# ERGO-Code/ipx

Hardware: AMD Instinct MI355X
Metric: kkt_solves_per_sec (higher is better)
Workload: dtype f64; 1 GPU; C3 synthetic LP m=1000000 n=2000000 8 nnz/col (nnz=16000000), KKTSolverDiag::Solve = diag-precond CR to tol=0.3*sqrt(mu), scaling spread s=1; rows of AI partitioned over 1 GPU(s); errflag=0

## Files before the change

ipx_amd/csrc/internal.hpp:

```cpp
#pragma once

#include <hip/hip_runtime.h>

#include <chrono>
#include <cstdint>
#include <cstdio>
#include <cstdlib>
#include <algorithm>
#include <cstring>
#include <functional>
#include <memory>
#include <stdexcept>
#include <string>
#include <type_traits>
#include <vector>

#include "../../include/ipx_kkt_hip.h"

namespace ipxk {

struct Error : std::runtime_error {
    int code;
    Error(int c, const std::string& what) : std::runtime_error(what), code(c) {}
};
// ... 77 lines not shown
    int64_t g = (n + kBlock - 1) / kBlock;
    if (g < 1) g = 1;
    return (int)(g < cap ? g : cap);
}
inline int vec_grid(int64_t len) { return grid_for(len, 1024); }

struct GatherView {
    int nrows, ncols;
    int P, G, RT, Q;
    int RWrows;
    const int* step_ptr;
    const int* wg_chunk_ptr;
    const int* chunk_start;
    const int* chunk_info;
    const int* chunk_step;
    const unsigned char* counts;
    const int* idx;
    const double* val;
    const unsigned char* row_long;
    int nseg;
    const int* seg_p0;
    const int* seg_p1;
    const int* lidx;
    const double* lval;
    int nlong;
    const int* long_row;
    const int* long_slot;
    double* long_partials;
    unsigned long long* stamps;
    int masked;
};

constexpr int kSlicedRows = 1024;
constexpr int kSlicedMaxTile = 7680;

struct SlicedView {
    int nrows, nrows_pad, nslices, nrb;
    int R;
    const unsigned* tile_ptr;
    const unsigned char* cnt;
    const int* idx;
    const double* val;
    double* partial;
    const unsigned char* row_long;
    int masked;
};

struct SlicedMatrix {
    bool built = false;
    int nslices = 0, nrb = 0, nrows_pad = 0, max_tile = 0, R = kSlicedRows;
    double dominant_fraction = 1.0;
    DevBuf<unsigned> tile_ptr;
    DevBuf<unsigned char> cnt;
    DevBuf<int> idx;
    DevBuf<double> val, partial;
};

constexpr int kSortedThreads = 256;
constexpr int kSortedMaxSub = 8192;
constexpr int kSortedOffBits = 18;
struct SortedView {
    int nrows, nrows_pad, nslices, nsub, nrb, RB, slice_elems;
    const int* xmin;
    const unsigned char* row_long;
    const unsigned* sub_ptr;
    const unsigned char* cnt;
    const unsigned* pack;
    const double* val;
    double* partial;
};
struct SortedMatrix {
    bool built = false;
    int nslices = 0, nsub = 0, nrb = 0, RB = 0, nrows_pad = 0, max_sub = 0, slice_elems = 0;
    DevBuf<unsigned> sub_ptr, pack;
    DevBuf<unsigned char> cnt;
    DevBuf<double> val, partial;
    bool fused = false;
    DevBuf<int> xmin;
};

constexpr int kAccThreads = 512;
constexpr int kAccPerThread = 4;
constexpr int kAccBatch = kAccThreads * kAccPerThread;
constexpr int kAccMaxRows = 16384;
struct AccView {
    int nrows, nrows_pad, nslices, nrb, RB, slice_elems;
    const int* xmin;
    const unsigned* tile_batch;
    const unsigned* bptr;
    const unsigned* pack;
    const double* val;
    double* partial;
};
struct AccMatrix {
    bool built = false;
    int nslices = 0, nrb = 0, RB = 0, nrows_pad = 0, slice_elems = 0;
    int64_t nbatches = 0, deferred = 0;
    DevBuf<unsigned> tile_batch, bptr, pack;
    DevBuf<double> val, partial;
    bool fused = false;
    DevBuf<int> xmin;
};

struct LayoutScratch;

enum class SpmvLayout { phased, sliced, fused, sorted, sortedfused, acc, plain, accfused };
constexpr int kNumSpmvLayouts = 8;
inline constexpr const char* kSpmvLayoutNames[kNumSpmvLayouts] = {"phased", "sliced", "fused", "sorted", "sortedfused", "acc", "plain",
                                                                  "accfused"};

inline int combine_grid_for(int64_t nrows) {
    static const int cap = [] { const char* e = getenv("IPXK_COMBINE_GRID"); return e && atoi(e) > 0 ? std::min(atoi(e), 1024) : 1024; }();
    return (int)std::min<int64_t>(cap, std::max<int64_t>(1, (nrows + kBlock - 1) / kBlock));
}

struct GatherMatrix {
    int nrows = 0, ncols = 0;
    int64_t nnz = 0;
    int P = 1, G = 1, RT = 1, Q = 1, RWrows = kBlock;
    DevBuf<int> step_ptr, idx, wg_chunk_ptr, chunk_start, chunk_info, chunk_step;
    DevBuf<unsigned char> counts, row_long;
    DevBuf<double> val;
    int nseg = 0, nlong = 0;
    DevBuf<int> seg_p0, seg_p1, lidx, long_row, long_slot;
    DevBuf<double> lval, long_partials;
    DevBuf<unsigned long long> stamps;
    int tune_level = 2;
    bool keep_plain = false;
    std::vector<int> h_plain_ptr;
    DevBuf<int> plain_idx;
    DevBuf<double> plain_val;

    void build(int64_t nrows_, int64_t ncols_, const ipxint* hptr, const ipxint* hidx,
               const double* hval, hipStream_t s);
    bool build_device(LayoutScratch& S, int64_t nrows_, int64_t ncols_, int64_t nnz_, const int* dptr, const int* didx,
                      const double* dval, hipStream_t s);
    bool build_device_local(LayoutScratch& S, int64_t nrows_, int64_t ncols_, int64_t nnz_, const int* dptr, const int* didx,
                            const double* dval, double share, hipStream_t s);
    void set_geometry(int64_t nrows_, int64_t ncols_);
    SpmvLayout layout = SpmvLayout::phased;
    SpmvLayout tile_base() const { return !sliced.built ? SpmvLayout::phased : sliced.nslices == 1 ? SpmvLayout::fused : SpmvLayout::sliced; }
    float tuned_us[kNumSpmvLayouts] = {};
    float time_layout(SpmvLayout L, hipStream_t s);
    void select_layout(const std::function<bool(SpmvLayout)>& make, hipStream_t s);
    SlicedMatrix sliced;
    SortedMatrix sorted;
    void build_sorted(const ipxint* hptr, const ipxint* hidx, const double* hval, hipStream_t s);
    void build_sorted_fused(const ipxint* hptr, const ipxint* hidx, const double* hval, hipStream_t s);
    AccMatrix acc;
    void build_acc(const ipxint* hptr, const ipxint* hidx, const double* hval, hipStream_t s);
    void build_acc_fused(const ipxint* hptr, const ipxint* hidx, const double* hval, hipStream_t s);
    AccMatrix accf;
    AccView acc_fused_view() const;
    AccView acc_view() const;
    const int* csr_ptr = nullptr;
    const int* csr_idx = nullptr;
    const double* csr_val = nullptr;
    int plain_grid() const { return (int)std::min<int64_t>(kMaxPartials, std::max<int64_t>(1, ((int64_t)nrows * 8 + kBlock - 1) / kBlock)); }
    int sorted_fused_grid() const {
        static const int cap = [] { const char* e = getenv("IPXK_SF_GRID"); return e && atoi(e) > 0 ? std::min(atoi(e), kMaxPartials) : kMaxPartials; }();
        return std::min(sorted.nrb, cap);
    }
    SortedView sorted_view() const;
    void build_sliced(const ipxint* hptr, const ipxint* hidx, const double* hval, hipStream_t s, int ns_request);
    SlicedView sliced_view(int which = 0) const;
    int fused_grid() const { return std::min(sliced.nrb, kMaxPartials); }
// ... 154 lines not shown
```

ipx_amd/csrc/layout_device.hip:

```cpp
#include <numeric>
#include <rocprim/device/device_radix_sort.hpp>
#include <rocprim/device/device_scan.hpp>

#include "layout_scratch.hpp"

namespace ipxk {

template <class K>
void sort_pairs(Tmp& T, const K* kin, K* kout, const unsigned* vin, unsigned* vout, size_t n, int bits, hipStream_t s) {
    size_t bytes = 0;
    IPXK_HIP(rocprim::radix_sort_pairs(nullptr, bytes, kin, kout, vin, vout, n, 0u, (unsigned)bits, s));
    IPXK_HIP(rocprim::radix_sort_pairs(T.need(bytes), bytes, kin, kout, vin, vout, n, 0u, (unsigned)bits, s));
}
template void sort_pairs<unsigned>(Tmp&, const unsigned*, unsigned*, const unsigned*, unsigned*, size_t, int, hipStream_t);
template void sort_pairs<u64>(Tmp&, const u64*, u64*, const unsigned*, unsigned*, size_t, int, hipStream_t);
void sort_keys(Tmp& T, u64* in, u64* out, size_t n, hipStream_t s) {
    size_t bytes = 0;
    IPXK_HIP(rocprim::radix_sort_keys(nullptr, bytes, in, out, n, 0u, 64u, s));
    IPXK_HIP(rocprim::radix_sort_keys(T.need(bytes), bytes, in, out, n, 0u, 64u, s));
}
void scan_int(Tmp& T, const int* in, int* out, size_t n, hipStream_t s) {
    size_t bytes = 0;
    IPXK_HIP(rocprim::exclusive_scan(nullptr, bytes, in, out, 0, n, rocprim::plus<int>(), s));
    IPXK_HIP(rocprim::exclusive_scan(T.need(bytes), bytes, in, out, 0, n, rocprim::plus<int>(), s));
// ... 99 lines not shown
                                u64* __restrict__ key, unsigned* __restrict__ pos, int* __restrict__ rowof) {
    IPXK_GRID_STRIDE(r, nrows) {
        const u64 tile0 = (u64)(r / RB) * (u64)ns;
        for (int p = ptr[r]; p < ptr[r + 1]; p++) {
            const int sl = idx[p] / slice, off = idx[p] - sl * slice;
            key[p] = ((tile0 + (u64)sl) << kSortedOffBits) | (u64)(unsigned)off;
            pos[p] = (unsigned)p;
            rowof[p] = (int)r;
        }
    }
}
__global__ void acc_words_kernel(int64_t nz, const u64* __restrict__ keys, const unsigned* __restrict__ perm, const int* __restrict__ rowof, int RB,
                                 unsigned* __restrict__ word) {
    IPXK_GRID_STRIDE(e, nz) word[e] = ((unsigned)(rowof[perm[e]] % RB) << kSortedOffBits) | (unsigned)(keys[e] & ((1u << kSortedOffBits) - 1u));
}
__global__ __launch_bounds__(64) void acc_batch_kernel(int RB, const unsigned* __restrict__ tile_ptr, const unsigned* __restrict__ word,
                                                        unsigned* __restrict__ dst, unsigned* pendA, unsigned* pendB, unsigned* __restrict__ bstart,
                                                        unsigned* __restrict__ nbatch, u64* deferred_total) {
    extern __shared__ unsigned ab_lds[];
    unsigned* stamp = ab_lds;
    unsigned* claim = ab_lds + RB;
    const int tile = blockIdx.x, lane = threadIdx.x;
    const unsigned e0 = tile_ptr[tile];
    const int ne = (int)(tile_ptr[tile + 1] - e0);
    for (int r = lane; r < RB; r += 64) { stamp[r] = 0u; claim[r] = 0xffffffffu; }
    __syncthreads();
    unsigned cur = 1;
    int fill = 0, out = 0, nb = 0, cursor = 0, na = 0, ia = 0, nbp = 0;
    u64 ndef = 0;
    unsigned *pa = pendA + e0, *pb = pendB + e0;
    if (ne > 0) { if (lane == 0) bstart[e0] = e0; nb = 1; }
    const u64 lt = (1ull << lane) - 1ull;
    while (out < ne) {
        int n = 0, c = 0;
        if (ia < na) {
            n = min(64, na - ia);
            if (lane < n) c = (int)__hip_atomic_load(pa + ia + lane, __ATOMIC_RELAXED, __HIP_MEMORY_SCOPE_AGENT);
            ia += n;
        } else if (fill < kAccBatch && cursor < ne) {
            n = min(64, ne - cursor);
            c = cursor + lane;
            cursor += n;
        } else {
            if (lane == 0) bstart[e0 + nb] = e0 + (unsigned)out;
            nb++; cur++; fill = 0;
            unsigned* t = pa; pa = pb; pb = t;
            na = nbp; ia = 0; nbp = 0;
            __syncthreads();
            continue;
        }
        const bool live = lane < n;
        const unsigned row = live ? (word[e0 + c] >> kSortedOffBits) : 0u;
        const bool ok = live && stamp[row] != cur;
        if (ok) atomicMin(&claim[row], (unsigned)lane);
        __syncthreads();
        const bool win = ok && claim[row] == (unsigned)lane;
        __syncthreads();
        if (win) { claim[row] = 0xffffffffu; stamp[row] = cur; }
        const u64 wmask = __ballot(win);
        const int prefix = __popcll(wmask & lt);
        const bool take = win && prefix < kAccBatch - fill;
        if (take) dst[e0 + c] = e0 + (unsigned)(out + prefix);
        const int nt = __popcll(__ballot(take));
        const bool def = live && !take;
        const u64 dmask = __ballot(def);
        if (def) pb[nbp + __popcll(dmask & lt)] = (unsigned)c;
        const int nd = __popcll(dmask);
        nbp += nd; ndef += (u64)nd; out += nt; fill += nt;
        __syncthreads();
    }
    if (lane == 0) {
        nbatch[tile] = (unsigned)nb;
        if (ndef) atomicAdd(deferred_total, ndef);
    }
}
__global__ void acc_scatter_kernel(int64_t nz, const unsigned* __restrict__ dst, const unsigned* __restrict__ word, const unsigned* __restrict__ perm,
                                   const double* __restrict__ val, unsigned* __restrict__ pack, double* __restrict__ out_val) {
    IPXK_GRID_STRIDE(e, nz) {
        const unsigned d = dst[e];
        pack[d] = word[e];
        out_val[d] = val[perm[e]];
    }
}
__global__ void acc_bptr_kernel(int ntiles, const unsigned* __restrict__ tile_ptr, const unsigned* __restrict__ tile_batch,
                                const unsigned* __restrict__ bstart, unsigned nz, unsigned* __restrict__ bptr) {
    const int tile = blockIdx.x;
    if (tile >= ntiles) return;
    const unsigned e0 = tile_ptr[tile], b0 = tile_batch[tile], nb = tile_batch[tile + 1] - b0;
    for (unsigned q = threadIdx.x; q < nb; q += blockDim.x) bptr[b0 + q] = bstart[e0 + q];
    if (tile == ntiles - 1 && threadIdx.x == 0) bptr[tile_batch[ntiles]] = nz;
}

__global__ void tile_window_kernel(int nrows, const int* __restrict__ ptr, const int* __restrict__ idx, int RB, int* __restrict__ lo,
                                   int* __restrict__ hi, unsigned char* __restrict__ cnt, int* flags) {
    IPXK_GRID_STRIDE(r, nrows) {
        const int p0 = ptr[r], p1 = ptr[r + 1];
        if (cnt) { if (p1 - p0 > 255) flags[0] = 1; cnt[r] = (unsigned char)(p1 - p0); }
        if (p1 == p0) continue;
        int a = idx[p0], b = a;
        for (int p = p0 + 1; p < p1; p++) {
            const int v = idx[p];
            if (v <= idx[p - 1]) flags[1] = 1;
            a = min(a, v); b = max(b, v);
        }
        atomicMin(lo + r / RB, a);
        atomicMax(hi + r / RB, b);
    }
}
__global__ void tile_window_stats_kernel(int nrb, int nrows, int RB, const int* __restrict__ ptr, int* __restrict__ lo, const int* __restrict__ hi,
                                         int* out) {
    IPXK_GRID_STRIDE(t, nrb) {
        const int r0 = (int)t * RB, r1 = min(nrows, r0 + RB);
        const int ne = ptr[r1] - ptr[r0];
        if (ne == 0) { lo[t] = 0; continue; }
        atomicMax(out + 0, hi[t] - lo[t]);
        atomicMax(out + 1, ne);
    }
}
__global__ void fused_keys_kernel(int nrows, const int* __restrict__ ptr, const int* __restrict__ idx, int RB, const int* __restrict__ lo,
                                  u64* __restrict__ key, unsigned* __restrict__ pos, int* __restrict__ rowof) {
    IPXK_GRID_STRIDE(r, nrows) {
        const u64 t = (u64)(r / RB);
        const int base = lo[r / RB];
        for (int p = ptr[r]; p < ptr[r + 1]; p++) {
            key[p] = (t << kSortedOffBits) | (u64)(unsigned)(idx[p] - base);
            pos[p] = (unsigned)p;
            if (rowof) rowof[p] = (int)r;
        }
    }
}
__global__ void sorted_fused_fill_kernel(int64_t nz, const u64* __restrict__ keys, const unsigned* __restrict__ perm, const int* __restrict__ ptr, int RB,
                                         const double* __restrict__ val, unsigned* __restrict__ pack, double* __restrict__ out_val) {
    IPXK_GRID_STRIDE(f, nz) {
        const u64 k = keys[f];
        const unsigned p = perm[f], t = (unsigned)(k >> kSortedOffBits);
        pack[f] = ((p - (unsigned)ptr[(size_t)t * RB]) << kSortedOffBits) | (unsigned)(k & ((1u << kSortedOffBits) - 1u));
        out_val[f] = val[p];
    }
}
__global__ void tile_ptr_from_rows_kernel(int nrb, int nrows, int RB, const int* __restrict__ ptr, unsigned* __restrict__ out) {
    IPXK_GRID_STRIDE(t, (int64_t)nrb + 1) out[t] = (unsigned)ptr[min((int64_t)nrows, t * RB)];
}
}

namespace {
constexpr int kMaxLongRowsDevice = 1 << 16;
__global__ void long_flag_kernel(int nrows, const int* __restrict__ ptr, unsigned char* __restrict__ flag, int* __restrict__ slen, int* counters,
                                 int* __restrict__ list, int cap) {
    IPXK_GRID_STRIDE(r, (int64_t)nrows + 1) {
        if (r == nrows) { slen[r] = 0; continue; }
        const int len = ptr[r + 1] - ptr[r];
        const bool lg = len > kMaxRowLen;
        flag[r] = lg ? 1 : 0;
        slen[r] = lg ? 0 : len;
        if (lg) {
            const int k = atomicAdd(counters, 1);
            if (k < cap) list[k] = (int)r;
        }
    }
}
__global__ void strip_copy_kernel(int nrows, const int* __restrict__ ptr, const int* __restrict__ sptr, const unsigned char* __restrict__ flag,
                                  const int* __restrict__ idx, const double* __restrict__ val, int* __restrict__ oidx, double* __restrict__ oval) {
    const int g = threadIdx.x & 7;
    for (int64_t r = ((int64_t)blockIdx.x * blockDim.x + threadIdx.x) >> 3; r < nrows; r += ((int64_t)gridDim.x * blockDim.x) >> 3) {
        if (flag[r]) continue;
        const int p0 = ptr[r], len = ptr[r + 1] - p0, q0 = sptr[r];
// ... 134 lines not shown
    for (;; search.next()) {
        RB = search.rows;
        if (search.gave_up()) return false;
        nrb = (nrows + RB - 1) / RB;
        nsubs = (int64_t)nrb * ns * nsub;
        if ((u64)nsubs * (u64)RB >= (u64(1) << 32)) return false;
        hipLaunchKernelGGL(sorted_keys1_kernel, dim3(gridn(nrows)), dim3(kBlock), 0, s, nrows, dptr, didx, RB, ns, nsub, (int)slice, (int)half,
                           S.k1.get(), S.v1.get());
        sort_pairs<unsigned>(S.T, S.k1.get(), S.k2.get(), S.v1.get(), S.v2.get(), nz, bits_for((u64)nsubs * (u64)RB - 1), s);
        out.sub_ptr.ensure((size_t)nsubs + 1);
        hipLaunchKernelGGL(lower_bounds_kernel<unsigned>, dim3(gridn(nsubs + 1)), dim3(kBlock), 0, s, nsubs + 1, nnz, S.k2.get(), (u64)RB, 0,
                           out.sub_ptr.get());
        IPXK_HIP(hipMemsetAsync(S.stats.get(), 0, 8 * sizeof(int), s));
        hipLaunchKernelGGL(max_range_kernel, dim3(gridn(nsubs)), dim3(kBlock), 0, s, nsubs, out.sub_ptr.get(), S.stats.get());
        IPXK_HIP(hipMemcpyAsync(&max_sub, S.stats.get(), sizeof(int), hipMemcpyDeviceToHost, s));
        IPXK_HIP(hipStreamSynchronize(s));
        if (search.fits(max_sub)) break;
    }
    const size_t nslots = (size_t)nsubs * RB;
    out.cnt.ensure(nslots); out.pack.ensure(nz); out.val.ensure(nz);
    IPXK_HIP(hipMemsetAsync(out.cnt.get(), 0, nslots, s));
    IPXK_HIP(hipMemsetAsync(S.stats.get(), 0, 8 * sizeof(int), s));
    hipLaunchKernelGGL(run_counts_kernel, dim3(gridn(nnz)), dim3(kBlock), 0, s, nnz, S.k2.get(), out.cnt.get(), S.stats.get());
    hipLaunchKernelGGL(sorted_keys2_kernel, dim3(gridn(nnz)), dim3(kBlock), 0, s, nnz, S.k2.get(), S.v2.get(), didx, RB, ns, nsub, (int)slice,
                       S.q1.get(), S.v3.get());
    sort_pairs<u64>(S.T, S.q1.get(), S.q2.get(), S.v3.get(), S.v4.get(), nz, kSortedOffBits + bits_for((u64)nsubs - 1), s);
    hipLaunchKernelGGL(sorted_fill_kernel, dim3(gridn(nnz)), dim3(kBlock), 0, s, nnz, S.q2.get(), S.v4.get(), S.v2.get(), out.sub_ptr.get(), dval,
                       out.pack.get(), out.val.get());
    int over = 0;
    IPXK_HIP(hipMemcpyAsync(&over, S.stats.get(), sizeof(int), hipMemcpyDeviceToHost, s));
    IPXK_HIP(hipStreamSynchronize(s));
    IPXK_HIP(hipGetLastError());
    if (over) { out = SortedMatrix(); return false; }
    out.nslices = ns; out.nsub = nsub; out.nrb = nrb; out.RB = RB; out.nrows_pad = nrb * RB;
    out.max_sub = max_sub; out.slice_elems = (int)slice;
    out.partial.resize((size_t)ns * out.nrows_pad);
    out.built = true;
    return true;
}

int acc_persist_grid(int ns) {
    static const int setting = [] { const char* e = getenv("IPXK_ACC_PERSIST"); return e ? std::max(0, atoi(e)) : 1; }();
    if (setting == 0 || ns < 1) return 0;
    static int cus[64] = {};
    int dev = 0;
    IPXK_HIP(hipGetDevice(&dev));
    if (dev < 0 || dev >= 64) dev = 0;
    if (cus[dev] == 0) IPXK_HIP(hipDeviceGetAttribute(&cus[dev], hipDeviceAttributeMultiprocessorCount, dev));
    const int L = std::lcm(8, ns);
    const int n = setting > 1 ? std::min(setting, cus[dev]) : cus[dev];
    return std::max(L, n / L * L);
}

int acc_rows_per_block(int nrows, int ns) {
    static const int cap = [] { const char* e = getenv("IPXK_ACC_ROWS"); return e && atoi(e) >= 1024 ? std::min(atoi(e), kAccMaxRows) & ~1 : kAccMaxRows; }();
    static const bool balance = !(getenv("IPXK_ACC_BALANCE") && getenv("IPXK_ACC_BALANCE")[0] == '0');
    if (const int G = balance ? acc_persist_grid(ns) : 0) {
        const int64_t per = G / ns;
        const int64_t nrb = (((int64_t)nrows + cap - 1) / cap + per - 1) / per * per;
        int rb = (int)(((int64_t)nrows + nrb - 1) / nrb);
        rb += rb & 1;
        if (rb >= 1024 && 8 * (int64_t)rb >= 7 * (int64_t)cap) return rb;
    }
    int RB = cap;
    while (RB > 1024 && ((int64_t)nrows + RB - 1) / RB * (int64_t)ns < 256) RB /= 2;
    return RB;
}

struct AccTemps {
    DevBuf<int> rowof;
    DevBuf<unsigned> tile_ptr, nbatch, bstart;
    AccTemps(int64_t ntiles, size_t nz) : rowof(nz), tile_ptr((size_t)ntiles + 1), nbatch((size_t)ntiles + 1), bstart(nz) {}
};
static void acc_batches(LayoutScratch& S, AccMatrix& out, AccTemps& T, int64_t ntiles, int RB, int64_t nnz, const double* dval, hipStream_t s) {
    const size_t nz = (size_t)nnz;
    unsigned* word = S.k1.get();
    hipLaunchKernelGGL(acc_words_kernel, dim3(gridn(nnz)), dim3(kBlock), 0, s, nnz, S.q2.get(), S.v2.get(), T.rowof.get(), RB, word);
    IPXK_HIP(hipMemsetAsync(S.stats.get(), 0, 8 * sizeof(int), s));
    const size_t lds = (size_t)RB * 2 * sizeof(unsigned);
    IPXK_HIP(hipFuncSetAttribute(reinterpret_cast<const void*>(acc_batch_kernel), hipFuncAttributeMaxDynamicSharedMemorySize,
                                 (int)(kAccMaxRows * 2 * sizeof(unsigned))));
    hipLaunchKernelGGL(acc_batch_kernel, dim3((unsigned)ntiles), dim3(64), lds, s, RB, T.tile_ptr.get(), word, S.k2.get(), S.v3.get(), S.v4.get(),
                       T.bstart.get(), T.nbatch.get(), reinterpret_cast<u64*>(S.stats.get()));
    out.tile_batch.ensure((size_t)ntiles + 1);
    scan_u32((int)ntiles, T.nbatch.get(), out.tile_batch.get(), s);
    unsigned nb_total = 0;
    u64 ndef = 0;
    IPXK_HIP(hipMemcpyAsync(&nb_total, out.tile_batch.get() + ntiles, sizeof(unsigned), hipMemcpyDeviceToHost, s));
    IPXK_HIP(hipMemcpyAsync(&ndef, S.stats.get(), sizeof(u64), hipMemcpyDeviceToHost, s));
    IPXK_HIP(hipStreamSynchronize(s));
    out.bptr.ensure((size_t)nb_total + 1); out.pack.ensure(nz); out.val.ensure(nz);
    hipLaunchKernelGGL(acc_bptr_kernel, dim3((unsigned)ntiles), dim3(64), 0, s, (int)ntiles, T.tile_ptr.get(), out.tile_batch.get(), T.bstart.get(),
                       (unsigned)nnz, out.bptr.get());
    hipLaunchKernelGGL(acc_scatter_kernel, dim3(gridn(nnz)), dim3(kBlock), 0, s, nnz, S.k2.get(), word, S.v2.get(), dval, out.pack.get(),
                       out.val.get());
    out.nbatches = nb_total; out.deferred = (int64_t)ndef;
}

static void tile_windows(LayoutScratch& S, int nrows, int nrb, int RB, const int* dptr, const int* didx, int* lo, int* hi, unsigned char* cnt,
                         int h[4], hipStream_t s) {
    IPXK_HIP(hipMemsetAsync(lo, 0x7f, (size_t)nrb * sizeof(int), s));
    IPXK_HIP(hipMemsetAsync(hi, 0xff, (size_t)nrb * sizeof(int), s));
    if (cnt) IPXK_HIP(hipMemsetAsync(cnt, 0, (size_t)nrb * RB, s));
    IPXK_HIP(hipMemsetAsync(S.stats.get(), 0, 8 * sizeof(int), s));
    hipLaunchKernelGGL(tile_window_kernel, dim3(gridn(nrows)), dim3(kBlock), 0, s, nrows, dptr, didx, RB, lo, hi, cnt, S.stats.get() + 2);
    hipLaunchKernelGGL(tile_window_stats_kernel, dim3(gridn(nrb)), dim3(kBlock), 0, s, nrb, nrows, RB, dptr, lo, hi, S.stats.get());
    IPXK_HIP(hipMemcpyAsync(h, S.stats.get(), 4 * sizeof(int), hipMemcpyDeviceToHost, s));
    IPXK_HIP(hipStreamSynchronize(s));
}

bool device_build_acc(LayoutScratch& S, AccMatrix& out, const SlicedMatrix& sliced, int nrows, int ncols, int64_t nnz, const int* dptr,
                      const int* didx, const double* dval, hipStream_t s) {
    out = AccMatrix();
    if (!sliced.built || sliced.nslices < 2 || nnz == 0) return false;
    const int ns = sliced.nslices;
    const int64_t slice = slice_width(ncols, ns);
    if (!offsets_fit(slice)) return false;
    const int RB = acc_rows_per_block(nrows, ns);
    const int nrb = (nrows + RB - 1) / RB;
    const int64_t ntiles = (int64_t)nrb * ns;
    const size_t nz = (size_t)nnz;
    S.q1.ensure(nz); S.q2.ensure(nz); S.v1.ensure(nz); S.v2.ensure(nz); S.v3.ensure(nz); S.v4.ensure(nz); S.k1.ensure(nz); S.k2.ensure(nz);
    S.stats.ensure(8);
    AccTemps T(ntiles, nz);
    hipLaunchKernelGGL(acc_keys_kernel, dim3(gridn(nrows)), dim3(kBlock), 0, s, nrows, dptr, didx, RB, ns, (int)slice, S.q1.get(), S.v1.get(), T.rowof.get());
    sort_pairs<u64>(S.T, S.q1.get(), S.q2.get(), S.v1.get(), S.v2.get(), nz, kSortedOffBits + bits_for((u64)std::max<int64_t>(ntiles, 2) - 1), s);
    hipLaunchKernelGGL(lower_bounds_kernel<u64>, dim3(gridn(ntiles + 1)), dim3(kBlock), 0, s, ntiles + 1, nnz, S.q2.get(), (u64)1, kSortedOffBits,
                       T.tile_ptr.get());
    acc_batches(S, out, T, ntiles, RB, nnz, dval, s);
    IPXK_HIP(hipStreamSynchronize(s));
    IPXK_HIP(hipGetLastError());
    out.nslices = ns; out.nrb = nrb; out.RB = RB; out.nrows_pad = nrb * RB; out.slice_elems = (int)slice;
    out.partial.resize((size_t)ns * out.nrows_pad);
    out.built = true;
    return true;
}

bool device_build_sorted_fused(LayoutScratch& S, SortedMatrix& out, int nrows, int ncols, int64_t nnz, const int* dptr, const int* didx,
                               const double* dval, hipStream_t s) {
    out = SortedMatrix();
    if (nrows == 0 || nnz == 0 || ncols == 0) return false;
    const size_t nz = (size_t)nnz;
    S.q1.ensure(nz); S.q2.ensure(nz); S.v1.ensure(nz); S.v2.ensure(nz); S.stats.ensure(8);
    DevBuf<int> lo, hi;
    RowBlockSearch search = sorted_fused_rows(nrows);
    int RB = 0, nrb = 0, h[4] = {0, 0, 0, 0};
    for (;; search.next()) {
        RB = search.rows;
        if (search.gave_up()) return false;
        nrb = (nrows + RB - 1) / RB;
        lo.ensure((size_t)nrb); hi.ensure((size_t)nrb);
        out.cnt.ensure((size_t)nrb * RB);
        tile_windows(S, nrows, nrb, RB, dptr, didx, lo.get(), hi.get(), out.cnt.get(), h, s);
        if (h[2]) { out = SortedMatrix(); return false; }
        if (search.fits(h[1])) break;
    }
    if (!window_fits(h[0])) { out = SortedMatrix(); return false; }
    hipLaunchKernelGGL(fused_keys_kernel, dim3(gridn(nrows)), dim3(kBlock), 0, s, nrows, dptr, didx, RB, lo.get(), S.q1.get(), S.v1.get(), (int*)nullptr);
    sort_pairs<u64>(S.T, S.q1.get(), S.q2.get(), S.v1.get(), S.v2.get(), nz, kSortedOffBits + bits_for((u64)std::max(nrb, 2) - 1), s);
    out.sub_ptr.ensure((size_t)nrb + 1); out.pack.ensure(nz); out.val.ensure(nz); out.xmin.ensure((size_t)nrb);
    hipLaunchKernelGGL(tile_ptr_from_rows_kernel, dim3(gridn(nrb + 1)), dim3(kBlock), 0, s, nrb, nrows, RB, dptr, out.sub_ptr.get());
    hipLaunchKernelGGL(sorted_fused_fill_kernel, dim3(gridn(nnz)), dim3(kBlock), 0, s, nnz, S.q2.get(), S.v2.get(), dptr, RB, dval, out.pack.get(), out.val.get());
    IPXK_HIP(hipMemcpyAsync(out.xmin.get(), lo.get(), (size_t)nrb * sizeof(int), hipMemcpyDeviceToDevice, s));
    IPXK_HIP(hipStreamSynchronize(s));
    IPXK_HIP(hipGetLastError());
    out.nslices = 1; out.nsub = 1; out.nrb = nrb; out.RB = RB; out.nrows_pad = nrb * RB; out.max_sub = h[1]; out.slice_elems = 0; out.fused = true;
    out.built = true;
    return true;
}

bool device_build_acc_fused(LayoutScratch& S, AccMatrix& out, int nrows, int ncols, int64_t nnz, const int* dptr, const int* didx,
                            const double* dval, hipStream_t s) {
    out = AccMatrix();
    if (nrows == 0 || nnz == 0 || ncols == 0) return false;
    const int RB = acc_fused_rows(nrows);
    if (RB == 0) return false;
    const int nrb = (nrows + RB - 1) / RB;
    const size_t nz = (size_t)nnz;
// ... 23 lines not shown
```

ipx_amd/csrc/layout_host.hip:

```cpp
#include <algorithm>
#include <cstdio>
#include <cstdlib>
#include <utility>

#include "context.hpp"

namespace ipxk {

void GatherMatrix::build(int64_t nrows_, int64_t ncols_, const ipxint* hptr, const ipxint* hidx,
                         const double* hval, hipStream_t s) {
    IPXK_REQUIRE(nrows_ >= 0 && ncols_ >= 0, "negative dimension");
    IPXK_REQUIRE(nrows_ < (int64_t(1) << 31) - 1 && ncols_ < (int64_t(1) << 31) - 1,
                 "dimension exceeds 32-bit device indices");
    const int64_t nz = hptr[nrows_];
    IPXK_REQUIRE(nz < (int64_t(1) << 31) - kLongSeg, "nnz exceeds 32-bit device indices");
    nrows = (int)nrows_;
    ncols = (int)ncols_;
    nnz = nz;

    set_geometry(nrows_, ncols_);
    const int64_t slice = phase_slice(ncols_);
    const int64_t RW = (int64_t)kBlock * RT;
    const int64_t nsteps = (int64_t)Q * P * G;
    IPXK_REQUIRE(nsteps * RW < (int64_t(1) << 40), "matrix too large for the phased layout");
// ... 212 lines not shown
    const bool verbose = getenv("IPXK_VERBOSE") != nullptr;
    RowBlockSearch search = sorted_rows();
    int RB = 0, nrb = 0, max_sub = 0;
    int64_t nsubs = 0, nshort = 0;
    std::vector<unsigned> sptr;
    std::vector<unsigned char> cnt;
    for (;; search.next()) {
        RB = search.rows;
        if (search.gave_up()) {
            if (verbose) fprintf(stderr, "ipxk: sorted layout not used for %d x %d: a sub-tile of %d rows holds %d entries\n", nrows, ncols, 2 * RB, max_sub);
            return;
        }
        nrb = (nrows + RB - 1) / RB;
        nsubs = (int64_t)nrb * ns * nsub;
        sptr.assign((size_t)nsubs + 1, 0);
        cnt.assign((size_t)nsubs * RB, 0);
        bool ok = true;
        for (int r = 0; r < nrows && ok; r++) {
            if (!rlong.empty() && rlong[r]) continue;
            const int64_t tile0 = (int64_t)(r / RB) * ns;
            for (ipxint p = hptr[r]; p < hptr[r + 1]; p++) {
                const int64_t sl = hidx[p] / slice, off = hidx[p] - sl * slice;
                const int64_t sub = (tile0 + sl) * nsub + std::min<int64_t>(off / half, nsub - 1);
                unsigned char& cc = cnt[(size_t)sub * RB + r % RB];
                if (cc == 255) { ok = false; break; }
                cc++;
                sptr[sub + 1]++;
            }
        }
        if (!ok) return;
        max_sub = 0;
        for (int64_t t = 0; t < nsubs; t++) { max_sub = std::max(max_sub, (int)sptr[t + 1]); sptr[t + 1] += sptr[t]; }
        nshort = sptr[nsubs];
        if (search.fits(max_sub)) break;
    }
    if (nshort == 0) return;
    std::vector<unsigned> pk((size_t)nshort);
    std::vector<double> tv((size_t)nshort);
    {
        std::vector<unsigned> cursor(sptr.begin(), sptr.end() - 1);
        for (int r = 0; r < nrows; r++) {
            if (!rlong.empty() && rlong[r]) continue;
            const int64_t tile0 = (int64_t)(r / RB) * ns;
            for (ipxint p = hptr[r]; p < hptr[r + 1]; p++) {
                const int64_t sl = hidx[p] / slice, off = hidx[p] - sl * slice;
                const int64_t sub = (tile0 + sl) * nsub + std::min<int64_t>(off / half, nsub - 1);
                const unsigned put = cursor[sub]++;
                pk[put] = ((put - sptr[sub]) << kSortedOffBits) | (unsigned)off;
                tv[put] = hval[p];
            }
        }
        std::vector<std::pair<unsigned, double>> tmp;
        const unsigned mask = (1u << kSortedOffBits) - 1u;
        for (int64_t t = 0; t < nsubs; t++) {
            const unsigned a = sptr[t], b = sptr[t + 1];
            if (b - a < 2) continue;
            tmp.resize(b - a);
            for (unsigned e = a; e < b; e++) tmp[e - a] = {pk[e], tv[e]};
            std::sort(tmp.begin(), tmp.end(), [&](const std::pair<unsigned, double>& x, const std::pair<unsigned, double>& y) {
                const unsigned ox = x.first & mask, oy = y.first & mask;
                return ox != oy ? ox < oy : x.first < y.first;
            });
            for (unsigned e = a; e < b; e++) { pk[e] = tmp[e - a].first; tv[e] = tmp[e - a].second; }
        }
    }
    sorted.nslices = ns; sorted.nsub = nsub; sorted.nrb = nrb; sorted.RB = RB; sorted.nrows_pad = nrb * RB;
    sorted.max_sub = max_sub; sorted.slice_elems = (int)slice;
    sorted.sub_ptr.upload(sptr, s);
    sorted.cnt.upload(cnt, s);
    sorted.pack.upload(pk, s);
    sorted.val.upload(tv, s);
    sorted.partial.resize((size_t)ns * sorted.nrows_pad);
    IPXK_HIP(hipStreamSynchronize(s));
    sorted.built = true;
}

namespace {
struct AccEntry { unsigned off, row; double v; };
struct AccBatcher {
    std::vector<unsigned> pk, bp;
    std::vector<double> tv;
    int64_t deferred = 0;
    std::vector<int> stamp, pend, newpend;
    AccBatcher(int64_t nnz, int RB) : pk((size_t)nnz), tv((size_t)nnz), stamp((size_t)RB) {}
    void tile(AccEntry* a, int ne, unsigned base) {
        std::stable_sort(a, a + ne, [](const AccEntry& x, const AccEntry& y) { return x.off < y.off; });
        std::fill(stamp.begin(), stamp.end(), -1);
        pend.clear();
        int cursor = 0, put = 0, batch = 0;
        while (put < ne) {
            bp.push_back(base + (unsigned)put);
            newpend.clear();
            int fill = 0;
            auto offer = [&](int i) {
                if (stamp[a[i].row] == batch || fill == kAccBatch) { newpend.push_back(i); deferred++; return; }
                stamp[a[i].row] = batch;
                pk[base + put] = (a[i].row << kSortedOffBits) | a[i].off;
                tv[base + put] = a[i].v;
                put++; fill++;
            };
            for (int i : pend) offer(i);
            while (fill < kAccBatch && cursor < ne) offer(cursor++);
            pend.swap(newpend);
            batch++;
        }
    }
    void finish(AccMatrix& A, std::vector<unsigned>& tb, int64_t nnz, hipStream_t s) {
        tb.back() = (unsigned)bp.size();
        bp.push_back((unsigned)nnz);
        A.nbatches = (int64_t)bp.size() - 1; A.deferred = deferred;
        A.tile_batch.upload(tb, s);
        A.bptr.upload(bp, s);
        A.pack.upload(pk, s);
        A.val.upload(tv, s);
    }
};
}

void GatherMatrix::build_acc(const ipxint* hptr, const ipxint* hidx, const double* hval, hipStream_t s) {
    acc = AccMatrix();
    if (!sliced.built || sliced.nslices < 2 || nlong > 0 || nnz == 0) return;
    const int ns = sliced.nslices;
    const int64_t slice = slice_width(ncols, ns);
    if (!offsets_fit(slice)) return;
    const int RB = acc_rows_per_block(nrows, ns);
    const int nrb = (nrows + RB - 1) / RB;
    const int64_t ntiles = (int64_t)nrb * ns;
    std::vector<unsigned> tptr((size_t)ntiles + 1, 0);
    for (int r = 0; r < nrows; r++)
        for (ipxint p = hptr[r]; p < hptr[r + 1]; p++) tptr[(size_t)(r / RB) * ns + hidx[p] / slice + 1]++;
    for (int64_t t = 0; t < ntiles; t++) tptr[t + 1] += tptr[t];
    std::vector<AccEntry> all((size_t)nnz);
    {
        std::vector<unsigned> cursor(tptr.begin(), tptr.end() - 1);
        for (int r = 0; r < nrows; r++)
            for (ipxint p = hptr[r]; p < hptr[r + 1]; p++) {
                const int64_t sl = hidx[p] / slice;
                all[cursor[(size_t)(r / RB) * ns + sl]++] = AccEntry{(unsigned)(hidx[p] - sl * slice), (unsigned)(r % RB), hval[p]};
            }
    }
    std::vector<unsigned> tb((size_t)ntiles + 1, 0);
    AccBatcher B(nnz, RB);
    for (int64_t t = 0; t < ntiles; t++) {
        tb[t] = (unsigned)B.bp.size();
        B.tile(all.data() + tptr[t], (int)(tptr[t + 1] - tptr[t]), tptr[t]);
    }
    acc.nslices = ns; acc.nrb = nrb; acc.RB = RB; acc.nrows_pad = nrb * RB; acc.slice_elems = (int)slice;
    B.finish(acc, tb, nnz, s);
    acc.partial.resize((size_t)ns * acc.nrows_pad);
    IPXK_HIP(hipStreamSynchronize(s));
    acc.built = true;
}

void GatherMatrix::build_acc_fused(const ipxint* hptr, const ipxint* hidx, const double* hval, hipStream_t s) {
    accf = AccMatrix();
    if (nrows == 0 || nnz == 0 || ncols == 0 || nlong > 0) return;
    for (int r = 0; r < nrows; r++)
        for (ipxint p = hptr[r] + 1; p < hptr[r + 1]; p++)
            if (hidx[p] <= hidx[p - 1]) return;
    const int RB = acc_fused_rows(nrows);
    if (RB == 0) return;
    const int nrb = (nrows + RB - 1) / RB;
    std::vector<AccEntry> a;
    std::vector<unsigned> tb((size_t)nrb + 1, 0);
    std::vector<int> xmin((size_t)nrb, 0);
    AccBatcher B(nnz, RB);
    unsigned base = 0;
    for (int t = 0; t < nrb; t++) {
        const int r1 = std::min(nrows, (t + 1) * RB);
        ipxint lo = ncols, hi = -1;
        for (int r = t * RB; r < r1; r++)
            for (ipxint p = hptr[r]; p < hptr[r + 1]; p++) { lo = std::min(lo, hidx[p]); hi = std::max(hi, hidx[p]); }
        tb[t] = (unsigned)B.bp.size();
        if (hi < 0) continue;
        if (!window_fits(hi - lo)) return;
        xmin[t] = (int)lo;
        a.clear();
        for (int r = t * RB; r < r1; r++)
            for (ipxint p = hptr[r]; p < hptr[r + 1]; p++) a.push_back(AccEntry{(unsigned)(hidx[p] - lo), (unsigned)(r - t * RB), hval[p]});
        B.tile(a.data(), (int)a.size(), base);
        base += (unsigned)a.size();
    }
    accf.nslices = 1; accf.nrb = nrb; accf.RB = RB; accf.nrows_pad = nrb * RB; accf.slice_elems = 0; accf.fused = true;
    B.finish(accf, tb, nnz, s);
    accf.xmin.upload(xmin, s);
    IPXK_HIP(hipStreamSynchronize(s));
    accf.built = true;
// ... 72 lines not shown
```

Measured before the change: 59.55 solves/s.

## Dissolve small trailing accumulation batches by migrating entries into earlier batches

Adds a post-pass, on both the device and host layout builders, that removes a tile's last batch when it holds at most a small cap of entries. Each tail entry is moved into the previous batch, using a chain of swaps so no row appears twice within a batch. The aim is fewer batches per tile, which means fewer per-batch synchronisations and partial-sum passes in the accumulate SpMV used by the CR solve. The cost is a more complex layout build, and the device kernel relies on relaxed atomics and a shared last-batch table whose correctness is delicate.

```diff
diff --git a/ipx_amd/csrc/internal.hpp b/ipx_amd/csrc/internal.hpp
--- a/ipx_amd/csrc/internal.hpp
+++ b/ipx_amd/csrc/internal.hpp
@@ -183,6 +183,7 @@
 constexpr int kAccThreads = 512;
 constexpr int kAccPerThread = 4;
 constexpr int kAccBatch = kAccThreads * kAccPerThread;
+constexpr int kAccTailCap = 64;
 constexpr int kAccMaxRows = 16384;
 struct AccView {
     int nrows, nrows_pad, nslices, nrb, RB, slice_elems;
diff --git a/ipx_amd/csrc/layout_device.hip b/ipx_amd/csrc/layout_device.hip
--- a/ipx_amd/csrc/layout_device.hip
+++ b/ipx_amd/csrc/layout_device.hip
@@ -205,6 +205,90 @@
         out_val[d] = val[perm[e]];
     }
 }
+__device__ inline unsigned tail_word(const unsigned* p) { return __hip_atomic_load(p, __ATOMIC_RELAXED, __HIP_MEMORY_SCOPE_AGENT); }
+__device__ inline void tail_move(unsigned* pack, u64* val, unsigned to, unsigned from) {
+    const unsigned w = tail_word(pack + from);
+    const u64 v = __hip_atomic_load(val + from, __ATOMIC_RELAXED, __HIP_MEMORY_SCOPE_AGENT);
+    __hip_atomic_store(pack + to, w, __ATOMIC_RELAXED, __HIP_MEMORY_SCOPE_AGENT);
+    __hip_atomic_store(val + to, v, __ATOMIC_RELAXED, __HIP_MEMORY_SCOPE_AGENT);
+}
+__device__ inline unsigned tail_find(const unsigned* pack, unsigned a, unsigned b, unsigned row, const unsigned* last, int lane) {
+    for (unsigned p = a; p < b; p += 64) {
+        const unsigned i = p + (unsigned)lane;
+        bool hit = false;
+        if (i < b) {
+            const unsigned r = tail_word(pack + i) >> kSortedOffBits;
+            hit = last ? last[r] == row : r == row;
+        }
+        const u64 m = __ballot(hit);
+        if (m) return p + (unsigned)__ffsll((unsigned long long)m) - 1u;
+    }
+    return ~0u;
+}
+__global__ __launch_bounds__(64) void acc_tail_kernel(const unsigned* __restrict__ tile_ptr, unsigned* bstart, unsigned* __restrict__ nbatch,
+                                                       unsigned* pack, double* val_) {
+    extern __shared__ unsigned at_last[];
+    u64* val = reinterpret_cast<u64*>(val_);
+    const int tile = blockIdx.x, lane = threadIdx.x;
+    const unsigned e0 = tile_ptr[tile], end = tile_ptr[tile + 1], none = ~0u;
+    const int nfull = (int)((end - e0 + kAccBatch - 1) / kAccBatch);
+    unsigned* bs = bstart + e0;
+    int nb = (int)nbatch[tile];
+    const int nb0 = nb;
+    bool have_last = false, stuck = false;
+    unsigned cut = 0;
+    for (;;) {
+        const int L = nb - 1;
+        if (L < 2 || nb <= nfull) break;
+        cut = bs[L];
+        if (end - cut > (unsigned)kAccTailCap) break;
+        if (!have_last) {
+            for (int q = 0; q < nb; q++) {
+                const unsigned b = q < L ? bs[q + 1] : end;
+                for (unsigned p = bs[q] + (unsigned)lane; p < b; p += 64) at_last[pack[p] >> kSortedOffBits] = (unsigned)q;
+                __syncthreads();
+            }
+            have_last = true;
+        }
+        while (cut < end) {
+            const unsigned r = tail_word(pack + cut) >> kSortedOffBits;
+            if (cut - bs[L - 1] >= (unsigned)kAccBatch) { stuck = true; break; }
+            int j = L - 1;
+            for (; j >= 0; j--)
+                if (tail_find(pack, bs[j], j == L - 1 ? cut : bs[j + 1], r, nullptr, lane) == none) break;
+            if (j < 0) { stuck = true; break; }
+            if (j < L - 1) {
+                const unsigned pf = tail_find(pack, bs[j], bs[j + 1], (unsigned)j, at_last, lane);
+                if (pf == none) { stuck = true; break; }
+                const unsigned fw = tail_word(pack + pf);
+                const u64 fv = __hip_atomic_load(val + pf, __ATOMIC_RELAXED, __HIP_MEMORY_SCOPE_AGENT);
+                unsigned slot = pf;
+                for (int q = j + 1; q < L; q++) {
+                    const unsigned p = tail_find(pack, bs[q], q == L - 1 ? cut : bs[q + 1], r, nullptr, lane);
+                    if (p == none) break;
+                    if (lane == 0) tail_move(pack, val, slot, p);
+                    slot = p;
+                }
+                if (lane == 0) {
+                    tail_move(pack, val, slot, cut);
+                    __hip_atomic_store(pack + cut, fw, __ATOMIC_RELAXED, __HIP_MEMORY_SCOPE_AGENT);
+                    __hip_atomic_store(val + cut, fv, __ATOMIC_RELAXED, __HIP_MEMORY_SCOPE_AGENT);
+                    at_last[fw >> kSortedOffBits] = (unsigned)(L - 1);
+                }
+            }
+            if (lane == 0) at_last[r] = (unsigned)(L - 1);
+            cut++;
+            __threadfence();
+            __syncthreads();
+        }
+        if (stuck) break;
+        nb--;
+    }
+    if (lane == 0 && (stuck || nb != nb0)) {
+        if (stuck) bs[nb - 1] = cut;
+        nbatch[tile] = (unsigned)nb;
+    }
+}
 __global__ void acc_bptr_kernel(int ntiles, const unsigned* __restrict__ tile_ptr, const unsigned* __restrict__ tile_batch,
                                 const unsigned* __restrict__ bstart, unsigned nz, unsigned* __restrict__ bptr) {
     const int tile = blockIdx.x;
@@ -505,6 +589,13 @@
                                  (int)(kAccMaxRows * 2 * sizeof(unsigned))));
     hipLaunchKernelGGL(acc_batch_kernel, dim3((unsigned)ntiles), dim3(64), lds, s, RB, T.tile_ptr.get(), word, S.k2.get(), S.v3.get(), S.v4.get(),
                        T.bstart.get(), T.nbatch.get(), reinterpret_cast<u64*>(S.stats.get()));
+    out.pack.ensure(nz); out.val.ensure(nz);
+    hipLaunchKernelGGL(acc_scatter_kernel, dim3(gridn(nnz)), dim3(kBlock), 0, s, nnz, S.k2.get(), word, S.v2.get(), dval, out.pack.get(),
+                       out.val.get());
+    IPXK_HIP(hipFuncSetAttribute(reinterpret_cast<const void*>(acc_tail_kernel), hipFuncAttributeMaxDynamicSharedMemorySize,
+                                 (int)(kAccMaxRows * sizeof(unsigned))));
+    hipLaunchKernelGGL(acc_tail_kernel, dim3((unsigned)ntiles), dim3(64), (size_t)RB * sizeof(unsigned), s, T.tile_ptr.get(), T.bstart.get(),
+                       T.nbatch.get(), out.pack.get(), out.val.get());
     out.tile_batch.ensure((size_t)ntiles + 1);
     scan_u32((int)ntiles, T.nbatch.get(), out.tile_batch.get(), s);
     unsigned nb_total = 0;
@@ -512,11 +603,9 @@
     IPXK_HIP(hipMemcpyAsync(&nb_total, out.tile_batch.get() + ntiles, sizeof(unsigned), hipMemcpyDeviceToHost, s));
     IPXK_HIP(hipMemcpyAsync(&ndef, S.stats.get(), sizeof(u64), hipMemcpyDeviceToHost, s));
     IPXK_HIP(hipStreamSynchronize(s));
-    out.bptr.ensure((size_t)nb_total + 1); out.pack.ensure(nz); out.val.ensure(nz);
+    out.bptr.ensure((size_t)nb_total + 1);
     hipLaunchKernelGGL(acc_bptr_kernel, dim3((unsigned)ntiles), dim3(64), 0, s, (int)ntiles, T.tile_ptr.get(), out.tile_batch.get(), T.bstart.get(),
                        (unsigned)nnz, out.bptr.get());
-    hipLaunchKernelGGL(acc_scatter_kernel, dim3(gridn(nnz)), dim3(kBlock), 0, s, nnz, S.k2.get(), word, S.v2.get(), dval, out.pack.get(),
-                       out.val.get());
     out.nbatches = nb_total; out.deferred = (int64_t)ndef;
 }
 
diff --git a/ipx_amd/csrc/layout_host.hip b/ipx_amd/csrc/layout_host.hip
--- a/ipx_amd/csrc/layout_host.hip
+++ b/ipx_amd/csrc/layout_host.hip
@@ -318,11 +318,13 @@
     std::vector<double> tv;
     int64_t deferred = 0;
     std::vector<int> stamp, pend, newpend;
+    std::vector<unsigned> chain;
     AccBatcher(int64_t nnz, int RB) : pk((size_t)nnz), tv((size_t)nnz), stamp((size_t)RB) {}
     void tile(AccEntry* a, int ne, unsigned base) {
         std::stable_sort(a, a + ne, [](const AccEntry& x, const AccEntry& y) { return x.off < y.off; });
         std::fill(stamp.begin(), stamp.end(), -1);
         pend.clear();
+        const size_t b0 = bp.size();
         int cursor = 0, put = 0, batch = 0;
         while (put < ne) {
             bp.push_back(base + (unsigned)put);
@@ -339,6 +341,54 @@
             while (fill < kAccBatch && cursor < ne) offer(cursor++);
             pend.swap(newpend);
             batch++;
+        }
+        dissolve_tail(base, base + (unsigned)ne, b0);
+    }
+    void dissolve_tail(unsigned base, unsigned end, size_t b0) {
+        const unsigned none = ~0u;
+        const int nfull = (int)((end - base + kAccBatch - 1) / kAccBatch);
+        auto row_at = [&](unsigned p) { return pk[p] >> kSortedOffBits; };
+        auto find_row = [&](unsigned a, unsigned b, unsigned r) { for (unsigned p = a; p < b; p++) if (row_at(p) == r) return p; return none; };
+        auto move = [&](unsigned to, unsigned from) { pk[to] = pk[from]; tv[to] = tv[from]; };
+        std::vector<int>& last = stamp;
+        bool have_last = false;
+        for (;;) {
+            const int nb = (int)(bp.size() - b0), L = nb - 1;
+            if (L < 2 || nb <= nfull) return;
+            unsigned* bs = bp.data() + b0;
+            if (end - bs[L] > (unsigned)kAccTailCap) return;
+            if (!have_last) {
+                for (int q = 0; q < nb; q++)
+                    for (unsigned p = bs[q]; p < (q < L ? bs[q + 1] : end); p++) last[row_at(p)] = q;
+                have_last = true;
+            }
+            while (bs[L] < end) {
+                const unsigned pe = bs[L], r = row_at(pe);
+                if (bs[L] - bs[L - 1] >= (unsigned)kAccBatch) return;
+                chain.clear();
+                int j = L - 1;
+                for (; j >= 0; j--) {
+                    const unsigned p = find_row(bs[j], bs[j + 1], r);
+                    if (p == none) break;
+                    chain.push_back(p);
+                }
+                if (j < 0) return;
+                if (j < L - 1) {
+                    unsigned pf = none;
+                    for (unsigned p = bs[j]; p < bs[j + 1] && pf == none; p++) if (last[row_at(p)] == j) pf = p;
+                    if (pf == none) return;
+                    const unsigned fw = pk[pf];
+                    const double fv = tv[pf];
+                    unsigned slot = pf;
+                    for (size_t k = chain.size(); k-- > 0; slot = chain[k]) move(slot, chain[k]);
+                    move(slot, pe);
+                    pk[pe] = fw; tv[pe] = fv;
+                    last[fw >> kSortedOffBits] = L - 1;
+                }
+                last[r] = L - 1;
+                bs[L]++;
+            }
+            bp.pop_back();
         }
     }
     void finish(AccMatrix& A, std::vector<unsigned>& tb, int64_t nnz, hipStream_t s) {
```

Measured after the change: 58.28 solves/s. 2.1% lower.
